# xiao-er-shang-jiu/Genie-TTS

Hardware: AMD Instinct MI355X
Metric: real-time factor + utterances/sec, 20-char JP, V2 speaker, 1/2/4/8 MI355X (higher is better)
Workload: dtype f32 activations (fp16-valued weights; split-fp16 MFMA GEMMs); 1 GPU; configs[1]: V2 speaker, single utterance, greedy, 1 utt per replica; a stream of such utterances, each one's vocoder on 64 CUs beside the next one's T2S; ref_phones=48, text_phones=45, ssl_frames=264, loop_steps=81, samples=102400, parallelism=replicas x1, vocoder_cus=64, streams_per_gpu=1, vits_f32_reruns=0

## Files before the change

genie_tts_amd/csrc/engine.hip:

```cpp
#include <hip/hip_runtime.h>
#include <hip/hip_fp16.h>

#include <chrono>
#include <cmath>
#include <cstdio>
#include <cstdlib>
#include <cstring>
#include <mutex>
#include <thread>
#include <map>
#include <memory>
#include <string>
#include <vector>

#include "../../include/genie_engine.h"
#include "engine_internal.h"
#include "kernels.h"
#include "prefill_attn.h"

using namespace gsv;

static thread_local std::string g_err;

const char* gsv_last_error(void) { return g_err.c_str(); }
// ... 265 lines not shown
}

int gsv_engine::finalize_t2s() {
    int err = 0;
    std::vector<float> div = default_div_term();
    if (const Staged* s = find("pe.div_term"))
        if (s->data.size() == 256) div = s->data;
    pe_max = 4096;
    if (const char* e = std::getenv("GENIE_FFN_SLICES")) ffn_slices = std::atoi(e) == 32 ? 32 : 64;
    if (const char* e = std::getenv("GENIE_ACC")) use_acc = std::atoi(e) != 0;
    if (const char* e = std::getenv("GENIE_PERSIST")) use_persist = std::atoi(e) != 0;
    if (const char* e = std::getenv("GENIE_PERSIST1")) use_persist1 = std::atoi(e) != 0;
    if (const char* e = std::getenv("GENIE_PERSIST1M")) use_persist1m = std::atoi(e) != 0;
    if (const char* e = std::getenv("GENIE_PERSISTM")) use_persistm = std::atoi(e) != 0;
    if (const char* e = std::getenv("GENIE_PRESPLIT")) use_presplit = std::atoi(e) != 0;
    if (const char* e = std::getenv("GENIE_CONVH")) use_convh = std::atoi(e) != 0;
    if (const char* e = std::getenv("GENIE_CONVH_WS")) convh_ws = std::max(0, std::min(2, std::atoi(e)));
    if (const char* e = std::getenv("GENIE_VITS_FORK")) vits_fork = std::atoi(e) != 0;
    if (const char* e = std::getenv("GENIE_PF_DELAY")) persist1_pf_delay = std::max(0, std::atoi(e));
    if (const char* e = std::getenv("GENIE_KTRACE"))
        if (std::atoi(e) == 1 && !ktrace) {
            hipMalloc(&ktrace, (size_t)3 * 256 * 8 * 8);
            hipMemset(ktrace, 0, (size_t)3 * 256 * 8 * 8);
        }
    std::vector<float> pe((size_t)pe_max * 512);
    for (int p = 0; p < pe_max; ++p)
        for (int i = 0; i < 256; ++i) {
            const float ang = (float)p * div[i];
            pe[(size_t)p * 512 + 2 * i] = std::sin(ang);
            pe[(size_t)p * 512 + 2 * i + 1] = std::cos(ang);
// ... 184 lines not shown
    e_h = A((size_t)cp * 768 * 4);
    e_hh = A((size_t)cp * 4);
    e_dist = A((size_t)cp * 1024 * 4);
    e_bproj = A((size_t)cl * 512 * 4);
    e_bert = A((size_t)cl * 1024 * 4);
    if (!e_im2col || !e_h || !e_hh || !e_dist || !e_bproj || !e_bert) return set_error(GSV_E_HIP, "encoder workspace");
    enc_cap_p = cp;
    enc_cap_l = cl;
    return 0;
}

int gsv_engine::encode(const gsv_utt* u, float* x, int64_t* prompts, hipStream_t st, bool do_prompts) {
    const int L = u->n_ref + u->n_text, P = u->n_ssl / 2;
    if (L <= 0 || P <= 0) return set_error(GSV_E_ARG, "empty utterance");
    if (int e = ensure_enc_ws(P, L)) return e;
    if (do_prompts) {
    ssl_im2col(u->ssl, u->n_ssl, e_im2col, st);
    GemmArgs g{};
    g.M = P; g.N = 768; g.K = 1536;
    g.A = e_im2col; g.lda = 1536;
    g.W = ssl_w; g.ldw = 1536; g.w_f16 = 0;
    g.bias = ssl_b; g.C = e_h; g.ldc = 768; g.mode = EPI_STORE;
    gemm_nt(g, st);
    sumsq_rows(e_h, 768, P, 768, e_hh, st);
    GemmArgs d{};
    d.M = P; d.N = 1024; d.K = 768;
    d.A = e_h; d.lda = 768; d.W = codebook; d.ldw = 768; d.w_f16 = 0;
    d.C = e_dist; d.ldc = 1024; d.mode = EPI_VQDIST; d.rowsq = e_hh; d.colsq = cb_sumsq;
    gemm_nt(d, st);
    argmin_dist_rows(e_dist, P, 1024, prompts, st);
    }
    const float* bproj = nullptr;
    if (u->ref_bert || u->text_bert) {
        if (u->ref_bert)
            hipMemcpyAsync(e_bert, u->ref_bert, (size_t)u->n_ref * 1024 * 4, hipMemcpyDeviceToDevice, st);
        else
            hipMemsetAsync(e_bert, 0, (size_t)u->n_ref * 1024 * 4, st);
        if (u->text_bert)
            hipMemcpyAsync(e_bert + (size_t)u->n_ref * 1024, u->text_bert, (size_t)u->n_text * 1024 * 4,
                           hipMemcpyDeviceToDevice, st);
        else
            hipMemsetAsync(e_bert + (size_t)u->n_ref * 1024, 0, (size_t)u->n_text * 1024 * 4, st);
        GemmArgs b{};
        b.M = L; b.N = 512; b.K = 1024;
        b.A = e_bert; b.lda = 1024; b.W = bert_w; b.ldw = 1024; b.w_f16 = 0;
        b.C = e_bproj; b.ldc = 512; b.mode = EPI_STORE;
        gemm_nt(b, st);
        bproj = e_bproj;
    }
    text_embed(u->ref_seq, u->n_ref, u->text_seq, u->n_text, text_emb, bproj, bert_b, alpha_text,
               pe_tab, x, st);
    const hipError_t le = hipGetLastError();
    return le == hipSuccess ? 0 : hip_error("encode launch", le);
}

int gsv_engine::prefill_slot(int b, const float* x, int L, const int64_t* pr, int P,
                             const gsv_sampler* sp, float* logits_out, hipStream_t st, int noise_b) {
    const int N0 = L + P;
    if (N0 + 1 > tmax) return set_error(GSV_E_CAPACITY, "prefill exceeds reserved tokens");
    if (x != pH) hipMemcpyAsync(pH, x, (size_t)L * 512 * 4, hipMemcpyDeviceToDevice, st);
    seq_state_init(b, pr, P, L, y, tmax, ny, kvlen, steps, done, seen, st);
    audio_embed_prompts(pr, P, emb_audio, alpha_audio, pe_tab, pH + (size_t)L * 512, st);
    hipLaunchKernelGGL(k_fill_row_len, dim3((N0 + 255) / 256), dim3(256), 0, st, prow_len, L, N0);
    const long sstride = (long)16 * tmax * 32;
    for (int l = 0; l < 24; ++l) {
        const T2SLayerW& W = layers[l];
        GemmArgs g{};
        g.M = N0; g.N = 1536; g.K = 512; g.A = pH; g.lda = 512;
        g.W = W.w_in; g.ldw = 512; g.w_f16 = 1; g.bias = W.b_in;
        g.C = pQ; g.ldc = 512; g.mode = EPI_QKV;
        g.kv.k = kcache[l] + b * sstride; g.kv.v = vcache[l] + b * sstride;
        g.kv.tmax = tmax; g.kv.pos0 = 0; g.kv.seq_stride = sstride;
        gemm_nt(g, st);
        AttnArgs at{};
        at.q = pQ; at.ldq = 512; at.k = kcache[l] + b * sstride; at.v = vcache[l] + b * sstride;
        at.seq_stride = sstride; at.tmax = tmax; at.row_len = prow_len; at.out = pO; at.ldo = 512;
        at.rows = N0; at.scale = qk_scale;
        attn_rows(at, st);
        const bool slabs = gemm_slabs_supported(512, 512, 512) && gemm_slabs_supported(2048, 2048, 2048);
        const long slab_stride = (long)tmax * 512;
        GemmArgs go{};
        go.M = N0; go.N = 512; go.K = 512; go.A = pO; go.lda = 512;
        go.W = W.w_out; go.ldw = 512; go.w_f16 = 1; go.bias = W.b_out;
        if (slabs) {
            go.C = pSlab; go.ldc = 512; go.mode = EPI_SLAB; go.ksplit = 4; go.slab_stride = slab_stride;
            gemm_nt(go, st);
            layernorm_rows_slabs(pSlab, 4, slab_stride, W.b_out, pH, pH1, N0, W.n1w, W.n1b, st);
        } else {
            go.C = pS; go.ldc = 512; go.mode = EPI_RESID; go.res = pH; go.ldr = 512;
            gemm_nt(go, st);
            layernorm_rows(pS, pH1, N0, W.n1w, W.n1b, st);
        }
        GemmArgs g1{};
        g1.M = N0; g1.N = 2048; g1.K = 512; g1.A = pH1; g1.lda = 512;
        g1.W = W.w1; g1.ldw = 512; g1.w_f16 = 1; g1.bias = W.b1;
        g1.C = pF; g1.ldc = 2048; g1.mode = EPI_RELU;
        gemm_nt(g1, st);
        GemmArgs g2{};
        g2.M = N0; g2.N = 512; g2.K = 2048; g2.A = pF; g2.lda = 2048;
        g2.W = W.w2; g2.ldw = 2048; g2.w_f16 = 1; g2.bias = W.b2;
        if (slabs) {
            g2.C = pSlab; g2.ldc = 512; g2.mode = EPI_SLAB; g2.ksplit = 8; g2.slab_stride = slab_stride;
            gemm_nt(g2, st);
            layernorm_rows_slabs(pSlab, 8, slab_stride, W.b2, pH1, pH, N0, W.n2w, W.n2b, st);
        } else {
            g2.C = pS; g2.ldc = 512; g2.mode = EPI_RESID; g2.res = pH1; g2.ldr = 512;
            gemm_nt(g2, st);
            layernorm_rows(pS, pH, N0, W.n2w, W.n2b, st);
        }
    }
    GemvArgs lg{};
    lg.B = 1; lg.N = 1025; lg.K = 512; lg.src = pH + (size_t)(N0 - 1) * 512; lg.lds = 512;
    lg.W = w_pred; lg.C = logits + (size_t)b * 1025; lg.ldc = 1025; lg.mode = EPI_STORE;
    gemv_f16(lg, st);
    SampleArgs sa = sampler_args(sp, 1);
// ... 1264 lines not shown
        if (value < 2) return set_error(GSV_E_ARG, "persistm_min_b: >= 2");
        eng->persistm_min_b = value;
    } else if (n == "persist_spin_ticks") {
        eng->persist_spin_ticks = value > 0 ? (unsigned long long)value : gsv_engine::PERSIST_SPIN_TICKS;
    } else if (n == "persist1_f16_limit") {
        eng->persist1_f16_limit = value;
    } else if (n == "pf_delay") {
        eng->persist1_pf_delay = std::max(0, value);
    } else if (n.size() == 5 && n.compare(0, 4, "knob") == 0 && n[4] >= '0' && n[4] <= '3') {
        eng->persist1_knob[n[4] - '0'] = value;
    } else if (n == "vits_lanes") {
        if (value < 1 || value > 16) return set_error(GSV_E_ARG, "vits_lanes: 1..16");
        eng->vits_lanes = value;
    } else if (n == "gemm_presplit") {
        eng->use_presplit = value != 0;
    } else if (n == "convh_ws") {
        eng->convh_ws = std::max(0, std::min(2, value));
    } else if (n == "vits_fork") {
        eng->vits_fork = value != 0;
    } else if (n == "vocoder_first") {
        eng->vocoder_first = value != 0;
    } else if (n == "lanes_all_cus") {
        if (int r = eng->vits_batch_finish(nullptr)) return r;
        eng->sync_own_streams();
        eng->lanes_all_cus = value != 0;
        if (int r = eng->remake_lane_streams()) return r;
    } else if (n == "lane_priority" || n == "t2s_priority") {
        int least = 0, greatest = 0;
        hipDeviceGetStreamPriorityRange(&least, &greatest);
        const int p = std::min(std::max(value, std::min(least, greatest)), std::max(least, greatest));
// ... 75 lines not shown
}

extern "C" int gsv_request_stop(gsv_engine* eng, int32_t on) {
    ENG_CHECK(eng);
    __atomic_store_n(eng->stop_word, on ? 1 : 0, __ATOMIC_RELEASE);
    return 0;
}

extern "C" int gsv_get_counter(gsv_engine* eng, const char* name, int64_t* value) {
    ENG_CHECK(eng);
    if (!name || !value) return set_error(GSV_E_ARG, "null arg");
    const std::string n(name);
    if (n == "persist_timeouts") *value = eng->persist_timeouts;
    else if (n == "persist1_f16_reruns") *value = eng->persist1_f16_reruns;
    else if (n == "vits_f32_reruns") *value = eng->vits_f32_reruns;
    else if (n == "vits_packed_fronts") *value = eng->vits_packed_fronts;
    else if (n == "sv_f32_reruns") *value = eng->sv_f32_reruns;
    else if (n == "w16_split_tensors") *value = eng->w16_split_tensors;
    else if (n == "persist_disabled") *value = eng->persist_disabled;
    else if (n == "persist_launches") *value = eng->persist_launches;
    else if (n == "decode_lanes") *value = eng->decode_lanes();
    else if (n == "lane_launches_0") *value = eng->lb.launches[0];
    else if (n == "lane_launches_1") *value = eng->lb.launches[1];
    else if (n == "persist_hold") *value = eng->persist_hold;
    else if (n == "stops") *value = eng->stops;
    else if (n == "graph_fallbacks") *value = eng->graph_fallbacks;
    else if (n == "retired_bytes") { std::lock_guard<std::mutex> g(eng->alloc_mu); *value = eng->retired_bytes; }
    else if (n == "reclaimed_bytes") *value = eng->reclaimed_bytes;
    else if (n == "reclaims") *value = eng->reclaims;
    else return set_error(GSV_E_ARG, "unknown counter " + n);
// ... 61 lines not shown
```

genie_tts_amd/csrc/engine_internal.h:

```cpp
#pragma once
#include <hip/hip_runtime.h>
#include <hip/hip_fp16.h>

#include <algorithm>
#include <map>
#include <mutex>
#include <shared_mutex>
#include <memory>
#include <thread>
#include <string>
#include <vector>

#include "../../include/genie_engine.h"
#include "kernels.h"
#include "lanes.h"
#include "vits.h"

namespace gsv {
int set_error(int code, const std::string& msg);
int check_sampler(const gsv_sampler* s);
inline float norm_top_p(float p) { return p == 0.f ? 1.f : p; }
int hip_error(const std::string& what, hipError_t e);
int f16_inexact_error(const std::string& weight, const float* v, int64_t index);
struct StreamScope;
// ... 192 lines not shown
    size_t sv_ws_floats(int frames);
    int sv_forward(const float* wav, int n, float* out, hipStream_t st, int* ovf, float lim);
    int roberta_forward(const int64_t* ids, int N, const int* rows, int n_out, float* out, hipStream_t st,
                        const int* row_pos = nullptr, const int* row_seg = nullptr);
    int reserve(int batch, int tokens);
    int ensure_enc_ws(int P, int L);
    int encode(const gsv_utt* u, float* x, int64_t* prompts, hipStream_t st, bool do_prompts = true);
    bool use_packed = true;
    bool use_attn_mf32 = true;
    int pk_rows = 0, pk_batch = 0;
    std::vector<void*> pk_allocs;
    float *pk_H = nullptr, *pk_Q = nullptr, *pk_O = nullptr, *pk_S = nullptr, *pk_H1 = nullptr, *pk_F = nullptr;
    float *pk_slab = nullptr, *pk_xlast = nullptr;
    __half *pk_Hh = nullptr, *pk_Hl = nullptr, *pk_H1h = nullptr, *pk_H1l = nullptr, *pk_Fh = nullptr, *pk_Fl = nullptr;
    bool use_presplit = true;
    int *pk_rowinfo = nullptr, *pk_last = nullptr;
    int64_t* pk_prompts = nullptr;
    int* pk_tiles = nullptr;
    int pk_tile_cap = 0;
    std::vector<int> pk_host;
    int ensure_packed(int rows, int B);
    int prefill_packed(int B, const gsv_utt* utts, const gsv_sampler* sp, hipStream_t st);
    int prefill_slot(int b, const float* x, int L, const int64_t* pr, int P, const gsv_sampler* sp,
                     float* logits_out, hipStream_t st, int noise_b = -1);
    gsv::SampleArgs sampler_args(const gsv_sampler* sp, int B);
    void decode_step(int B, const gsv_sampler* sp, float* logits_out, hipStream_t st);
    hipGraphExec_t step_graph(int B, const gsv_sampler* sp, int chunk, hipStream_t st);
    int decode_loop(int B, const gsv_sampler* sp, hipStream_t st, bool allow_persist = true);
    long persist_timeouts = 0;
    int persist_timeout_run = 0;
// ... 218 lines not shown
```

genie_tts_amd/csrc/kernels.h:

```cpp
#pragma once
#include <hip/hip_runtime.h>
#include <hip/hip_fp16.h>
#include <stdint.h>

namespace gsv {

enum EpiMode {
    EPI_STORE = 0,
    EPI_RELU = 1,
    EPI_RESID = 2,
    EPI_QKV = 3,
    EPI_VQDIST = 4,
    EPI_MISH = 5,
    EPI_SLAB = 6,
    EPI_GELU = 7,
    EPI_RELU_SPLIT = 8,
};

struct KVScatter {
    float* k;
    float* v;
    int tmax;
    int pos0;
    const int* row_pos;
// ... 12 lines not shown
struct GemmArgs {
    int M, N, K;
    const float* A; long lda;
    const void* W; long ldw; int w_f16;
    const void* Wl;
    const float* bias;
    float* C; long ldc;
    int mode;
    const float* res; long ldr;
    const float* rowsq; const float* colsq;
    KVScatter kv;
    int ksplit; long slab_stride;
    int a_nslab; long a_slab_stride; const float* a_bias; int a_relu;
    const __half* Ah; const __half* Al;
    __half* Ch; __half* Cl;
};
void gemm_nt(const GemmArgs& a, hipStream_t s);
GemmArgs gemm_f16(int M, int N, int K, const float* A, long lda, const void* W, const float* bias, float* C,
                  long ldc, int mode, const float* res = nullptr, long ldr = 0);
GemmArgs gemm_w16(int M, int N, int K, const float* A, long lda, const W16& W, const float* bias, float* C,
                  long ldc, int mode, const float* res = nullptr, long ldr = 0);
bool gemm_slabs_supported(int K, long lda, long ldw);
bool gemm_w16_supported(int K, long lda, long ldw);
bool gemm_presplit_path(int M, int N, int K, long lda);

void layernorm_rows(const float* in, float* out, int rows, const float* g, const float* b,
                    hipStream_t s);
void layernorm_rows_slabs(const float* slabs, int nsplit, long slab_stride, const float* bias,
                          const float* res, float* out, int rows, const float* g, const float* b,
                          hipStream_t s, __half* out_hi = nullptr, __half* out_lo = nullptr);
// ... 162 lines not shown
```

genie_tts_amd/csrc/t2s.hip:

```cpp
#include "common.h"
#include "kernels.h"
#include "prefill_attn.h"
#include "sampler.h"
#include <cstdio>
#include <cstdlib>

namespace gsv {

__device__ __forceinline__ void gemm_epilogue(const GemmArgs& a, int row0, int col, int lane, const f32x16& acc) {
    if (col >= a.N) return;
    const float bv = a.bias ? a.bias[col] : 0.f;
#pragma unroll
    for (int r = 0; r < 16; ++r) {
        const int row = row0 + (r & 3) + 8 * (r >> 2) + 4 * (lane >> 5);
        if (row >= a.M) continue;
        const float v = a.bias ? bv + acc[r] : acc[r];
        switch (a.mode) {
            case EPI_STORE: a.C[(long)row * a.ldc + col] = v; break;
            case EPI_RELU: a.C[(long)row * a.ldc + col] = fmaxf(v, 0.f); break;
            case EPI_RELU_SPLIT: {
                float x = fmaxf(v, 0.f);
                asm volatile("" : "+v"(x));
                const _Float16 h = (_Float16)x;
                reinterpret_cast<_Float16*>(a.Ch)[(long)row * a.ldc + col] = h;
// ... 343 lines not shown
        if (a.mode == EPI_SLAB) {
            if (col >= a.N) continue;
            float* C = a.C + (long)kz * a.slab_stride;
#pragma unroll
            for (int i = 0; i < 16; ++i) {
                const int row = m0 + wm * 32 + (i & 3) + 8 * (i >> 2) + 4 * hh;
                if (row < a.M) C[(long)row * a.ldc + col] = acc[t][i];
            }
            continue;
        }
        gemm_epilogue(a, m0 + wm * 32, col, lane, acc[t]);
    }
}

enum class X3Form { SplitW, LargeM, SmallM };
static void launch_x3(const GemmArgs& a, int z, hipStream_t s, X3Form form) {
    auto go = [&](auto kern) {
        hipLaunchKernelGGL(kern, dim3((a.N + 63) / 64, (a.M + 63) / 64, z), dim3(256), 0, s, a);
    };
    switch (form) {
        case X3Form::SplitW: go(k_gemm_x3<64, 64, 2, true, 1, true>); break;
        case X3Form::LargeM:
            if (a.Ah) go(k_gemm_x3<64, 64, 2, false, 1, true, true>);
            else go(k_gemm_x3<64, 64, 2, false, 1, true>);
            break;
        case X3Form::SmallM: go(k_gemm_x3<64, 64, 4>); break;
    }
}

static bool gemm_big(const GemmArgs& a) { return (long)((a.M + 63) / 64) * ((a.N + 63) / 64) >= 1024; }

bool gemm_w16_supported(int K, long lda, long ldw) { return K % GX_KS == 0 && lda % 4 == 0 && ldw % 8 == 0; }

bool gemm_presplit_path(int M, int N, int K, long lda) {
    if (K % GX_KS != 0 || lda % 8 != 0) return false;
    GemmArgs t{};
    t.M = M; t.N = N;
    return gemm_big(t);
}

bool gemm_slabs_supported(int K, long lda, long ldw) { return K % GX_KS == 0 && lda % 4 == 0 && ldw % 8 == 0; }
// ... 1010 lines not shown
```

genie_tts_amd/csrc/vits.h:

```cpp
#pragma once
#include <hip/hip_runtime.h>
#include <hip/hip_fp16.h>
#include <stdint.h>

#include <vector>

namespace gsv {

constexpr int MHA_MAXK_HOST = 2048;

enum ConvMode {
    CV_STORE = 0,
    CV_RELU = 1,
    CV_RESID = 2,
    CV_VEC = 3,
    CV_SUB = 4,
    CV_TANH = 5,
    CV_ACC_FIRST = 6,
    CV_ACC_ADD = 7,
    CV_ACC_MEAN = 8,
    CV_RESID_VEC = 9,
    CV_SPLIT_RESID = 10,
};

// ... 5 lines not shown
    int in_act; float in_slope;
    int mode;
    const float* res; long r_cs, r_ts;
    const float* vec;
    float* acc; float div;
    int split; float* out2; const float* res2;
    int phases; long w_phase_stride;
    float* part; long part_cap;
    const __half* wh; const float* wscale; int* ovf;
    long wh_phase_stride; const float* in_scale;
    const int* seg; long vec_sstride;
    int tile_force;
    int ws;
};
void conv1d(const ConvArgs& a, hipStream_t s);
void seg_fill(int* seg, long n, const int* off, const int* len, int nseg, int f, hipStream_t s);
bool conv1d_h(const ConvArgs& a, hipStream_t s);

struct MrfPairArgs {
    const float* r; int T, C, K, dil;
    const __half* w1; const float* s1; const float* b1;
    const __half* w2; const float* s2;
    int* ovf;
    ConvArgs e;
};
bool mrf_pair(const MrfPairArgs& a, hipStream_t s);

void mean3(const float* a, const float* b, const float* c, float* out, long n, float div, hipStream_t s);
void ln_channels(const float* x, const float* y, float* out, int C, int T, const float* g,
                 const float* b, hipStream_t s, const int* seg = nullptr);

struct MhaArgs {
    const float* q; long q_ts, q_cs;
    const float* k; long k_ts, k_cs;
    const float* v; long v_ts, v_cs;
    float* out; long o_ts, o_cs;
    int nq, nk, heads, dk;
    int postdiv; float scale;
    const float* ek; const float* ev; int window;
    const int* row_seg;
};
void mha(const MhaArgs& a, hipStream_t s);

void codebook_upsample2(const int64_t* sem, int G, const float* cb, float* out, hipStream_t s);
void embed_channels(const int64_t* ids, int n, const float* emb, int C, float* out, hipStream_t s);
void wn_gate(const float* xin, float* acts, int H, int T, hipStream_t s);
void glu_resid(const float* h, const float* x, float* out, int C, int T, long x_cs, long x_ts,
               hipStream_t s);
void noise_zp(const float* m, const float* logs, const float* eps, float scale, float* z, int n,
              hipStream_t s);
void noise_zp_philox(const float* m, const float* logs, uint64_t seed, float scale, float* z, int n,
                     hipStream_t s);
void flip_channels(const float* in, float* out, int C, int T, hipStream_t s);
void interp_linear(const float* x, int C, int T, int T_out, float* out, hipStream_t s);
void codebook_upsample2_seg(const int64_t* const* sems, const int* seg, const int* off, int T, const float* cb,
                            float* out, hipStream_t s);
void embed_channels_seg(const int64_t* const* ids, const int* seg, const int* off, int n, const float* emb, int C,
                        float* out, hipStream_t s);
void noise_zp_philox_seg(const float* m, const float* logs, const uint64_t* seeds, const int* seg, const int* off,
                         const int* len, float scale, float* z, int C, int T, hipStream_t s);
void gather_vecs(const float* const* ptrs, int n, int dim, float* out, hipStream_t s);
// ... 81 lines not shown
```

genie_tts_amd/csrc/vits.hip:

```cpp
#include "common.h"
#include "vits.h"
#include "vits_epi.h"
#include <algorithm>
#include <cstdlib>

namespace gsv {

template <int KT> struct ConvCfg {
    static constexpr int CI = KT == 1 ? 32 : KT == 2 ? 32 : KT <= 4 ? 16 : KT <= 7 ? 8 : 4;
    static constexpr int KC = CI * KT;
};

#define CONV_BN 64
#define CONV_BM 64
#define CONV_XW_MAX 128

template <int KT, bool V4>
__global__ __launch_bounds__(256) void k_conv1d(ConvArgs a) {
    constexpr int CI = ConvCfg<KT>::CI, KC = ConvCfg<KT>::KC;
    constexpr int NX = (CI * CONV_XW_MAX + 255) / 256;
    constexpr int NW = (CONV_BM * KC / 4 + 255) / 256;
    __shared__ float Xs[2][CI * CONV_XW_MAX];
    __shared__ float Ws[2][CONV_BM][KC + 1];
    const int tid = threadIdx.x, lane = tid & 63, w = tid >> 6;
// ... 135 lines not shown
    else hipLaunchKernelGGL((k_conv1d<KT, false>), grid, dim3(256), 0, s, a);
}

static int conv_ci(int K) {
    switch (K) {
        case 1: return ConvCfg<1>::CI;
        case 2: return ConvCfg<2>::CI;
        case 3: return ConvCfg<3>::CI;
        case 4: return ConvCfg<4>::CI;
        case 5: return ConvCfg<5>::CI;
        case 7: return ConvCfg<7>::CI;
        default: return ConvCfg<11>::CI;
    }
}

void conv1d(const ConvArgs& a, hipStream_t s) {
    if (a.wh && conv1d_h(a, s)) return;
    dim3 grid((a.n_t + CONV_BN - 1) / CONV_BN, (a.Cout + CONV_BM - 1) / CONV_BM,
              a.phases > 0 ? a.phases : 1);
    int nsplit = 1;
    const int blocks = (int)(grid.x * grid.y);
    if (a.part && a.phases <= 1 && blocks < 128) {
        const int nch = (a.Cin + conv_ci(a.K) - 1) / conv_ci(a.K);
        nsplit = std::min(nch, (256 + blocks - 1) / blocks);
        while (nsplit > 1 && (long)nsplit * a.Cout * a.n_t > a.part_cap) --nsplit;
    }
    if (nsplit > 1) grid.z = nsplit;
    switch (a.K) {
        case 1: launch_conv<1>(a, grid, s); break;
        case 2: launch_conv<2>(a, grid, s); break;
        case 3: launch_conv<3>(a, grid, s); break;
        case 4: launch_conv<4>(a, grid, s); break;
        case 5: launch_conv<5>(a, grid, s); break;
        case 7: launch_conv<7>(a, grid, s); break;
        case 11: launch_conv<11>(a, grid, s); break;
        default: return;
    }
    if (nsplit > 1) {
        const long n = (long)a.Cout * a.n_t;
        hipLaunchKernelGGL(k_conv_reduce, dim3((unsigned)((n + 255) / 256)), dim3(256), 0, s, a, nsplit);
    }
}

__global__ __launch_bounds__(256) void k_mean3(const float4* __restrict__ a, const float4* __restrict__ b,
                                                const float4* __restrict__ c, float4* __restrict__ o, long n4,
                                                float div) {
    const long i = (long)blockIdx.x * 256 + threadIdx.x;
    if (i >= n4) return;
    const float4 x = a[i], y = b[i], z = c[i];
    o[i] = make_float4(((x.x + y.x) + z.x) / div, ((x.y + y.y) + z.y) / div, ((x.z + y.z) + z.z) / div,
                       ((x.w + y.w) + z.w) / div);
}
__global__ __launch_bounds__(256) void k_mean3_tail(const float* a, const float* b, const float* c, float* o, long lo,
                                                     long n, float div) {
    const long i = lo + (long)blockIdx.x * 256 + threadIdx.x;
    if (i < n) o[i] = ((a[i] + b[i]) + c[i]) / div;
// ... 61 lines not shown
            const float d = v[i] - mean;
            q += d * d;
        }
    }
    red[cg][tl] = q;
    __syncthreads();
    const float den = sqrtf((red[0][tl] + red[1][tl] + red[2][tl] + red[3][tl]) / (float)C + 1e-5f);
    if (!ok) return;
#pragma unroll
    for (int i = 0; i < LNC_MAX; ++i) {
        const int c = cg + 4 * i;
        if (c < C) out[(long)c * T + t] = (v[i] - mean) / den * g[c] + b[c];
    }
}

__global__ __launch_bounds__(64) void k_ln_channels_w(const float* x, const float* y, float* out,
                                                     int C, int T, const float* g, const float* b,
                                                     const int* seg) {
    const int lane = threadIdx.x, tl = lane & 3, cg = lane >> 2;
    const int t = blockIdx.x * 4 + tl;
    const bool ok = t < T;
    const bool gap = ok && seg && seg[t] < 0;
    const int nc = C >> 4;
    float v[16];
    float s = 0.f;
#pragma unroll
    for (int i = 0; i < 16; ++i) {
        float xv = 0.f;
        if (i < nc && ok) {
            const long o = (long)(cg + 16 * i) * T + t;
            xv = x[o];
            if (y) xv = xv + y[o];
        }
        v[i] = xv;
        s += xv;
    }
#pragma unroll
    for (int o = 4; o < 64; o <<= 1) s += __shfl_xor(s, o, 64);
    const float mean = s / (float)C;
    float q = 0.f;
#pragma unroll
    for (int i = 0; i < 16; ++i)
        if (i < nc) {
            const float d = v[i] - mean;
            q += d * d;
        }
#pragma unroll
    for (int o = 4; o < 64; o <<= 1) q += __shfl_xor(q, o, 64);
    const float den = sqrtf(q / (float)C + 1e-5f);
    if (!ok) return;
#pragma unroll
    for (int i = 0; i < 16; ++i)
        if (i < nc) {
            const int c = cg + 16 * i;
            out[(long)c * T + t] = gap ? 0.f : (v[i] - mean) / den * g[c] + b[c];
        }
}

void ln_channels(const float* x, const float* y, float* out, int C, int T, const float* g,
                 const float* b, hipStream_t s, const int* seg) {
    if (C % 16 == 0 && C <= 256)
        hipLaunchKernelGGL(k_ln_channels_w, dim3((T + 3) / 4), dim3(64), 0, s, x, y, out, C, T, g, b, seg);
    else if (!seg)
        hipLaunchKernelGGL(k_ln_channels, dim3((T + 63) / 64), dim3(256), 0, s, x, y, out, C, T, g, b);
    else
        std::abort();
}

#define MHA_MAXK 2048
#define MHA_MAXD 128
#define MHA_MAXW 8
__global__ __launch_bounds__(256) void k_mha(MhaArgs a) {
    __shared__ float qs[MHA_MAXD];
    __shared__ float p[MHA_MAXK];
    __shared__ float red[16];
    __shared__ float part[2][MHA_MAXD];
    __shared__ float qe[2 * MHA_MAXW + 1];
    const int hd = blockIdx.x, i = blockIdx.y, tid = threadIdx.x;
    const int dk = a.dk, c0 = hd * dk;
    int nk = a.nk;
    const float* kb = a.k;
// ... 107 lines not shown
}
void embed_channels(const int64_t* ids, int n, const float* emb, int C, float* out, hipStream_t s) {
    hipLaunchKernelGGL(k_embed_ch, dim3((n + 127) / 128, C), dim3(128), 0, s, ids, n, emb, C, out);
}

__global__ void k_wn_gate(const float* xin, float* acts, int H, int T) {
    const long i = (long)blockIdx.x * blockDim.x + threadIdx.x;
    if (i >= (long)H * T) return;
    const float a = xin[i], b = xin[i + (long)H * T];
    acts[i] = tanhf(a) * (1.0f / (1.0f + expf(-b)));
}
void wn_gate(const float* xin, float* acts, int H, int T, hipStream_t s) {
    const long n = (long)H * T;
    hipLaunchKernelGGL(k_wn_gate, dim3((n + 255) / 256), dim3(256), 0, s, xin, acts, H, T);
}

__global__ void k_glu(const float* h, const float* x, float* out, int C, int T, long x_cs, long x_ts) {
    const long i = (long)blockIdx.x * blockDim.x + threadIdx.x;
    if (i >= (long)C * T) return;
    const int c = (int)(i / T), t = (int)(i - (long)c * T);
    const float a = h[i], b = h[i + (long)C * T];
    const long xi = (long)c * x_cs + (long)t * x_ts;
    out[xi] = x[xi] + a * (1.0f / (1.0f + expf(-b)));
}
void glu_resid(const float* h, const float* x, float* out, int C, int T, long x_cs, long x_ts,
               hipStream_t s) {
    const long n = (long)C * T;
    hipLaunchKernelGGL(k_glu, dim3((n + 255) / 256), dim3(256), 0, s, h, x, out, C, T, x_cs, x_ts);
}

// ... 178 lines not shown
```

genie_tts_amd/csrc/vits_engine.hip:

```cpp
#include <hip/hip_runtime.h>

#include <cmath>
#include <cstring>
#include <cstdlib>
#include <string>
#include <vector>

#include "engine_internal.h"

#include <thread>

using namespace gsv;

namespace {

std::vector<float> fold_wn(const Staged* v, const Staged* g) {
    const long o = v->dims[0];
    const long per = (long)v->data.size() / o;
    std::vector<float> w(v->data.size());
    for (long i = 0; i < o; ++i) {
        double s = 0;
        for (long j = 0; j < per; ++j) s += (double)v->data[i * per + j] * v->data[i * per + j];
        const float nrm = (float)std::sqrt(s);
        const float gg = g->data[i];
// ... 307 lines not shown
    a.x = x; a.x_cs = T; a.x_ts = 1; a.Cin = c.cin; a.Tin = T;
    a.w = c.w; a.Cout = c.cout; a.K = c.k; a.dil = 1; a.pad = (c.k - 1) / 2;
    a.bias = c.b;
    a.out = out; a.o_cs = T; a.o_ts = 1; a.n_t = T; a.o_tstride = 1; a.o_toff = 0; a.o_len = T;
    a.mode = mode; a.r_cs = T; a.r_ts = 1;
    a.phases = 1;
    a.tile_force = tls_convh_tile;
    a.ws = tls_convh_ws;
    if (tls_ovf && c.wh) { a.wh = c.wh; a.wscale = c.wscale; a.ovf = tls_ovf; }
    return a;
}

static void attn_encoder(gsv_engine* e, const std::vector<AttnLayer>& Ls, float* x, int T, float* qkv,
                         float* att, float* tmp, float* ffn, hipStream_t s, const int* seg = nullptr,
                         const int* rows = nullptr) {
    for (const AttnLayer& L : Ls) {
        conv1d(cargs(L.qkv, x, T, qkv, CV_STORE, seg), s);
        MhaArgs m{};
        m.q = qkv; m.q_ts = 1; m.q_cs = T;
        m.k = qkv + (size_t)192 * T; m.k_ts = 1; m.k_cs = T;
        m.v = qkv + (size_t)384 * T; m.v_ts = 1; m.v_cs = T;
        m.out = att; m.o_ts = 1; m.o_cs = T;
        m.nq = T; m.nk = T; m.heads = 2; m.dk = 96; m.postdiv = 0; m.scale = std::sqrt(96.0f);
        m.ek = L.ek; m.ev = L.ev; m.window = 4;
        m.row_seg = rows;
        mha(m, s);
        conv1d(cargs(L.o, att, T, tmp, CV_STORE, seg), s);
        ln_channels(x, tmp, x, 192, T, L.g1, L.b1, s, seg);
        conv1d(cargs(L.ffn1, x, T, ffn, CV_RELU, seg), s);
        conv1d(cargs(L.ffn2, ffn, T, tmp, CV_STORE, seg), s);
        ln_channels(x, tmp, x, 192, T, L.g2, L.b2, s, seg);
    }
}

static void run_ref_enc(VitsWorkspace& W, const RefEnc& R, const float* audio, int n, float* ge,
                        hipStream_t s) {
    const int padded = n + 2 * 704;
    const int F = (padded - 2048) / 640 + 1;
    reflect_pad(audio, n, 704, W.pad, s);
    GemmArgs g{};
    g.M = F; g.N = 1408; g.K = 2048; g.A = W.pad; g.lda = 640;
    g.W = R.dft; g.ldw = 2048; g.w_f16 = 0; g.C = W.reim; g.ldc = 1408; g.mode = EPI_STORE;
    gemm_nt(g, s);
    stft_mag(W.reim, F, 704, W.spec, s);
    GemmArgs l0{};
    l0.M = F; l0.N = 128; l0.K = 704; l0.A = W.spec; l0.lda = 704;
// ... 611 lines not shown
        a.x_cs = 1; a.x_ts = c.cin;
        a.o_cs = 1; a.o_ts = c.cout;
        conv1d(a, s);
    };
    float* gcond = fs ? fs->gcond : W.gcond;
    for (int fi = 3; fi >= 0; --fi) {
        const auto& fl = V.flows[fi];
        flip_channels(W.z, W.z2, 192, T, s);
        vec_conv(fl.cond, ge, gcond);
        conv1d(cargs(fl.pre, W.z2, T, W.fh, CV_STORE, sT), s);
        hipMemsetAsync(W.fskip, 0, (size_t)192 * T * 4, s);
        for (int l = 0; l < 4; ++l) {
            ConvArgs ci = cargs(fl.in_l[l], W.fh, T, W.fx, CV_VEC, sT);
            ci.vec = gcond + l * 384;
            ci.vec_sstride = fl.cond.cout;
            conv1d(ci, s);
            wn_gate(W.fx, W.fa, 192, T, s);
            if (l < 3) {
                ConvArgs rs = cargs(fl.rs[l], W.fa, T, W.fh, CV_SPLIT_RESID, sT);
                rs.res = W.fh; rs.split = 192; rs.out2 = W.fskip; rs.res2 = W.fskip;
                conv1d(rs, s);
            } else {
                ConvArgs rs = cargs(fl.rs[l], W.fa, T, W.fskip, CV_RESID, sT);
                rs.res = W.fskip;
                conv1d(rs, s);
            }
        }
        ConvArgs po = cargs(fl.post, W.fskip, T, W.z2 + (size_t)96 * T, CV_SUB, sT);
        po.res = W.z2 + (size_t)96 * T;
        conv1d(po, s);
        float* t = W.z; W.z = W.z2; W.z2 = t;
    }
// ... 603 lines not shown
```

Measured before the change: 119.0 utt/s.

## Fuse split-K conv reductions into LayerNorm and WN gate; CU-aware small-M GEMM staging

Split-K conv1d calls in the VITS attention encoder and flow WN layers can now defer their partial-slab reduction. New kernels sum the slabs, add the bias and apply LayerNorm or the tanh-sigmoid gate in one pass, which removes a separate reduce kernel launch and a round trip through the intermediate buffer. Separately, the small-M T2S prefill GEMMs now receive the stream's CU count and use a 2-stage pipeline instead of 4 when the block count exceeds the available CUs, with an env/knob override. The trade-offs are extra code paths and a different reduction order, which can change numerics slightly.

```diff
diff --git a/genie_tts_amd/csrc/engine.hip b/genie_tts_amd/csrc/engine.hip
--- a/genie_tts_amd/csrc/engine.hip
+++ b/genie_tts_amd/csrc/engine.hip
@@ -303,6 +303,11 @@
     if (const char* e = std::getenv("GENIE_PERSIST1M")) use_persist1m = std::atoi(e) != 0;
     if (const char* e = std::getenv("GENIE_PERSISTM")) use_persistm = std::atoi(e) != 0;
     if (const char* e = std::getenv("GENIE_PRESPLIT")) use_presplit = std::atoi(e) != 0;
+    if (const char* e = std::getenv("GENIE_GEMM_SMALL_NS")) {
+        const int v = std::atoi(e);
+        gemm_small_ns = v >= 2 && v <= 4 ? v : 0;
+    }
+    if (const char* e = std::getenv("GENIE_VITS_SLAB_FUSE")) vits_slab_fuse = std::atoi(e) != 0;
     if (const char* e = std::getenv("GENIE_CONVH")) use_convh = std::atoi(e) != 0;
     if (const char* e = std::getenv("GENIE_CONVH_WS")) convh_ws = std::max(0, std::min(2, std::atoi(e)));
     if (const char* e = std::getenv("GENIE_VITS_FORK")) vits_fork = std::atoi(e) != 0;
@@ -517,19 +522,20 @@
     const int L = u->n_ref + u->n_text, P = u->n_ssl / 2;
     if (L <= 0 || P <= 0) return set_error(GSV_E_ARG, "empty utterance");
     if (int e = ensure_enc_ws(P, L)) return e;
+    const int cus = stream_cus(st);
     if (do_prompts) {
     ssl_im2col(u->ssl, u->n_ssl, e_im2col, st);
     GemmArgs g{};
     g.M = P; g.N = 768; g.K = 1536;
     g.A = e_im2col; g.lda = 1536;
     g.W = ssl_w; g.ldw = 1536; g.w_f16 = 0;
-    g.bias = ssl_b; g.C = e_h; g.ldc = 768; g.mode = EPI_STORE;
+    g.bias = ssl_b; g.C = e_h; g.ldc = 768; g.mode = EPI_STORE; g.cus = cus;
     gemm_nt(g, st);
     sumsq_rows(e_h, 768, P, 768, e_hh, st);
     GemmArgs d{};
     d.M = P; d.N = 1024; d.K = 768;
     d.A = e_h; d.lda = 768; d.W = codebook; d.ldw = 768; d.w_f16 = 0;
-    d.C = e_dist; d.ldc = 1024; d.mode = EPI_VQDIST; d.rowsq = e_hh; d.colsq = cb_sumsq;
+    d.C = e_dist; d.ldc = 1024; d.mode = EPI_VQDIST; d.rowsq = e_hh; d.colsq = cb_sumsq; d.cus = cus;
     gemm_nt(d, st);
     argmin_dist_rows(e_dist, P, 1024, prompts, st);
     }
@@ -547,7 +553,7 @@
         GemmArgs b{};
         b.M = L; b.N = 512; b.K = 1024;
         b.A = e_bert; b.lda = 1024; b.W = bert_w; b.ldw = 1024; b.w_f16 = 0;
-        b.C = e_bproj; b.ldc = 512; b.mode = EPI_STORE;
+        b.C = e_bproj; b.ldc = 512; b.mode = EPI_STORE; b.cus = cus;
         gemm_nt(b, st);
         bproj = e_bproj;
     }
@@ -566,12 +572,14 @@
     audio_embed_prompts(pr, P, emb_audio, alpha_audio, pe_tab, pH + (size_t)L * 512, st);
     hipLaunchKernelGGL(k_fill_row_len, dim3((N0 + 255) / 256), dim3(256), 0, st, prow_len, L, N0);
     const long sstride = (long)16 * tmax * 32;
+    const int cus = stream_cus(st);
     for (int l = 0; l < 24; ++l) {
         const T2SLayerW& W = layers[l];
         GemmArgs g{};
         g.M = N0; g.N = 1536; g.K = 512; g.A = pH; g.lda = 512;
         g.W = W.w_in; g.ldw = 512; g.w_f16 = 1; g.bias = W.b_in;
         g.C = pQ; g.ldc = 512; g.mode = EPI_QKV;
+        g.cus = cus; g.small_ns = gemm_small_ns;
         g.kv.k = kcache[l] + b * sstride; g.kv.v = vcache[l] + b * sstride;
         g.kv.tmax = tmax; g.kv.pos0 = 0; g.kv.seq_stride = sstride;
         gemm_nt(g, st);
@@ -585,6 +593,7 @@
         GemmArgs go{};
         go.M = N0; go.N = 512; go.K = 512; go.A = pO; go.lda = 512;
         go.W = W.w_out; go.ldw = 512; go.w_f16 = 1; go.bias = W.b_out;
+        go.cus = cus; go.small_ns = gemm_small_ns;
         if (slabs) {
             go.C = pSlab; go.ldc = 512; go.mode = EPI_SLAB; go.ksplit = 4; go.slab_stride = slab_stride;
             gemm_nt(go, st);
@@ -598,10 +607,12 @@
         g1.M = N0; g1.N = 2048; g1.K = 512; g1.A = pH1; g1.lda = 512;
         g1.W = W.w1; g1.ldw = 512; g1.w_f16 = 1; g1.bias = W.b1;
         g1.C = pF; g1.ldc = 2048; g1.mode = EPI_RELU;
+        g1.cus = cus; g1.small_ns = gemm_small_ns;
         gemm_nt(g1, st);
         GemmArgs g2{};
         g2.M = N0; g2.N = 512; g2.K = 2048; g2.A = pF; g2.lda = 2048;
         g2.W = W.w2; g2.ldw = 2048; g2.w_f16 = 1; g2.bias = W.b2;
+        g2.cus = cus; g2.small_ns = gemm_small_ns;
         if (slabs) {
             g2.C = pSlab; g2.ldc = 512; g2.mode = EPI_SLAB; g2.ksplit = 8; g2.slab_stride = slab_stride;
             gemm_nt(g2, st);
@@ -1896,6 +1907,11 @@
         eng->vits_lanes = value;
     } else if (n == "gemm_presplit") {
         eng->use_presplit = value != 0;
+    } else if (n == "vits_slab_fuse") {
+        eng->vits_slab_fuse = value != 0;
+    } else if (n == "gemm_small_ns") {
+        if (value != 0 && (value < 2 || value > 4)) return set_error(GSV_E_ARG, "gemm_small_ns: 0, 2, 3 or 4");
+        eng->gemm_small_ns = value;
     } else if (n == "convh_ws") {
         eng->convh_ws = std::max(0, std::min(2, value));
     } else if (n == "vits_fork") {
@@ -2001,6 +2017,7 @@
     if (n == "persist_timeouts") *value = eng->persist_timeouts;
     else if (n == "persist1_f16_reruns") *value = eng->persist1_f16_reruns;
     else if (n == "vits_f32_reruns") *value = eng->vits_f32_reruns;
+    else if (n == "vits_slab_consumers") *value = eng->vits_slab_consumers.load();
     else if (n == "vits_packed_fronts") *value = eng->vits_packed_fronts;
     else if (n == "sv_f32_reruns") *value = eng->sv_f32_reruns;
     else if (n == "w16_split_tensors") *value = eng->w16_split_tensors;
diff --git a/genie_tts_amd/csrc/engine_internal.h b/genie_tts_amd/csrc/engine_internal.h
--- a/genie_tts_amd/csrc/engine_internal.h
+++ b/genie_tts_amd/csrc/engine_internal.h
@@ -1,4 +1,5 @@
 #pragma once
+#include <atomic>
 #include <hip/hip_runtime.h>
 #include <hip/hip_fp16.h>
 
@@ -230,6 +231,9 @@
     float *pk_slab = nullptr, *pk_xlast = nullptr;
     __half *pk_Hh = nullptr, *pk_Hl = nullptr, *pk_H1h = nullptr, *pk_H1l = nullptr, *pk_Fh = nullptr, *pk_Fl = nullptr;
     bool use_presplit = true;
+    std::atomic<long> vits_slab_consumers{0};
+    bool vits_slab_fuse = true;
+    int gemm_small_ns = 0;
     int *pk_rowinfo = nullptr, *pk_last = nullptr;
     int64_t* pk_prompts = nullptr;
     int* pk_tiles = nullptr;
diff --git a/genie_tts_amd/csrc/kernels.h b/genie_tts_amd/csrc/kernels.h
--- a/genie_tts_amd/csrc/kernels.h
+++ b/genie_tts_amd/csrc/kernels.h
@@ -50,6 +50,7 @@
     int a_nslab; long a_slab_stride; const float* a_bias; int a_relu;
     const __half* Ah; const __half* Al;
     __half* Ch; __half* Cl;
+    int cus, small_ns;
 };
 void gemm_nt(const GemmArgs& a, hipStream_t s);
 GemmArgs gemm_f16(int M, int N, int K, const float* A, long lda, const void* W, const float* bias, float* C,
diff --git a/genie_tts_amd/csrc/t2s.hip b/genie_tts_amd/csrc/t2s.hip
--- a/genie_tts_amd/csrc/t2s.hip
+++ b/genie_tts_amd/csrc/t2s.hip
@@ -381,6 +381,12 @@
 }
 
 enum class X3Form { SplitW, LargeM, SmallM };
+
+static int small_m_stages(const GemmArgs& a, long blocks) {
+    if (a.small_ns) return a.small_ns;
+    return a.cus > 0 && blocks > a.cus ? 2 : 4;
+}
+
 static void launch_x3(const GemmArgs& a, int z, hipStream_t s, X3Form form) {
     auto go = [&](auto kern) {
         hipLaunchKernelGGL(kern, dim3((a.N + 63) / 64, (a.M + 63) / 64, z), dim3(256), 0, s, a);
@@ -391,7 +397,16 @@
             if (a.Ah) go(k_gemm_x3<64, 64, 2, false, 1, true, true>);
             else go(k_gemm_x3<64, 64, 2, false, 1, true>);
             break;
-        case X3Form::SmallM: go(k_gemm_x3<64, 64, 4>); break;
+        case X3Form::SmallM:
+            switch (small_m_stages(a, (long)((a.N + 63) / 64) * ((a.M + 63) / 64) * z)) {
+                case 2: go(k_gemm_x3<64, 64, 2>); break;
+                case 3: go(k_gemm_x3<64, 64, 3>); break;
+                case 4: go(k_gemm_x3<64, 64, 4>); break;
+                default:
+                    std::fprintf(stderr, "gemm_nt: small-M ring depth %d\n", a.small_ns);
+                    std::abort();
+            }
+            break;
     }
 }
 
diff --git a/genie_tts_amd/csrc/vits.h b/genie_tts_amd/csrc/vits.h
--- a/genie_tts_amd/csrc/vits.h
+++ b/genie_tts_amd/csrc/vits.h
@@ -43,6 +43,7 @@
     int ws;
 };
 void conv1d(const ConvArgs& a, hipStream_t s);
+int conv1d_deferred(const ConvArgs& a, hipStream_t s);
 void seg_fill(int* seg, long n, const int* off, const int* len, int nseg, int f, hipStream_t s);
 bool conv1d_h(const ConvArgs& a, hipStream_t s);
 
@@ -58,6 +59,8 @@
 void mean3(const float* a, const float* b, const float* c, float* out, long n, float div, hipStream_t s);
 void ln_channels(const float* x, const float* y, float* out, int C, int T, const float* g,
                  const float* b, hipStream_t s, const int* seg = nullptr);
+void ln_channels_slabs(const float* x, const float* slabs, int nsplit, const float* bias, float* out, int C, int T,
+                       const float* g, const float* b, hipStream_t s, const int* seg = nullptr);
 
 struct MhaArgs {
     const float* q; long q_ts, q_cs;
@@ -74,6 +77,8 @@
 void codebook_upsample2(const int64_t* sem, int G, const float* cb, float* out, hipStream_t s);
 void embed_channels(const int64_t* ids, int n, const float* emb, int C, float* out, hipStream_t s);
 void wn_gate(const float* xin, float* acts, int H, int T, hipStream_t s);
+void wn_gate_slabs(const float* slabs, int nsplit, const float* bias, const float* vec, long vec_sstride,
+                   const int* seg, float* acts, int H, int T, hipStream_t s);
 void glu_resid(const float* h, const float* x, float* out, int C, int T, long x_cs, long x_ts,
                hipStream_t s);
 void noise_zp(const float* m, const float* logs, const float* eps, float scale, float* z, int n,
diff --git a/genie_tts_amd/csrc/vits.hip b/genie_tts_amd/csrc/vits.hip
--- a/genie_tts_amd/csrc/vits.hip
+++ b/genie_tts_amd/csrc/vits.hip
@@ -173,8 +173,8 @@
     }
 }
 
-void conv1d(const ConvArgs& a, hipStream_t s) {
-    if (a.wh && conv1d_h(a, s)) return;
+static int conv1d_run(const ConvArgs& a, hipStream_t s, bool defer) {
+    if (a.wh && conv1d_h(a, s)) return 1;
     dim3 grid((a.n_t + CONV_BN - 1) / CONV_BN, (a.Cout + CONV_BM - 1) / CONV_BM,
               a.phases > 0 ? a.phases : 1);
     int nsplit = 1;
@@ -193,12 +193,20 @@
         case 5: launch_conv<5>(a, grid, s); break;
         case 7: launch_conv<7>(a, grid, s); break;
         case 11: launch_conv<11>(a, grid, s); break;
-        default: return;
-    }
-    if (nsplit > 1) {
+        default: return 1;
+    }
+    if (nsplit > 1 && !defer) {
         const long n = (long)a.Cout * a.n_t;
         hipLaunchKernelGGL(k_conv_reduce, dim3((unsigned)((n + 255) / 256)), dim3(256), 0, s, a, nsplit);
     }
+    return nsplit;
+}
+
+void conv1d(const ConvArgs& a, hipStream_t s) { conv1d_run(a, s, false); }
+
+int conv1d_deferred(const ConvArgs& a, hipStream_t s) {
+    const int nsplit = conv1d_run(a, s, true);
+    return nsplit > 1 ? nsplit : 0;
 }
 
 __global__ __launch_bounds__(256) void k_mean3(const float4* __restrict__ a, const float4* __restrict__ b,
@@ -290,6 +298,34 @@
     }
 }
 
+__device__ __forceinline__ void ln_w_finish(const float (&v)[16], float* out, int C, int T, const float* g,
+                                            const float* b, int t, int cg, bool ok, bool gap, int i0, int di) {
+    const int nc = C >> 4;
+    float s = 0.f;
+#pragma unroll
+    for (int i = 0; i < 16; ++i) s += v[i];
+#pragma unroll
+    for (int o = 4; o < 64; o <<= 1) s += __shfl_xor(s, o, 64);
+    const float mean = s / (float)C;
+    float q = 0.f;
+#pragma unroll
+    for (int i = 0; i < 16; ++i)
+        if (i < nc) {
+            const float d = v[i] - mean;
+            q += d * d;
+        }
+#pragma unroll
+    for (int o = 4; o < 64; o <<= 1) q += __shfl_xor(q, o, 64);
+    const float den = sqrtf(q / (float)C + 1e-5f);
+    if (!ok) return;
+#pragma unroll
+    for (int i = 0; i < 16; ++i)
+        if (i < nc && i % di == i0) {
+            const int c = cg + 16 * i;
+            out[(long)c * T + t] = gap ? 0.f : (v[i] - mean) / den * g[c] + b[c];
+        }
+}
+
 __global__ __launch_bounds__(64) void k_ln_channels_w(const float* x, const float* y, float* out,
                                                      int C, int T, const float* g, const float* b,
                                                      const int* seg) {
@@ -299,7 +335,6 @@
     const bool gap = ok && seg && seg[t] < 0;
     const int nc = C >> 4;
     float v[16];
-    float s = 0.f;
 #pragma unroll
     for (int i = 0; i < 16; ++i) {
         float xv = 0.f;
@@ -309,28 +344,58 @@
             if (y) xv = xv + y[o];
         }
         v[i] = xv;
-        s += xv;
-    }
-#pragma unroll
-    for (int o = 4; o < 64; o <<= 1) s += __shfl_xor(s, o, 64);
-    const float mean = s / (float)C;
-    float q = 0.f;
-#pragma unroll
-    for (int i = 0; i < 16; ++i)
-        if (i < nc) {
-            const float d = v[i] - mean;
-            q += d * d;
-        }
-#pragma unroll
-    for (int o = 4; o < 64; o <<= 1) q += __shfl_xor(q, o, 64);
-    const float den = sqrtf(q / (float)C + 1e-5f);
-    if (!ok) return;
-#pragma unroll
-    for (int i = 0; i < 16; ++i)
-        if (i < nc) {
-            const int c = cg + 16 * i;
-            out[(long)c * T + t] = gap ? 0.f : (v[i] - mean) / den * g[c] + b[c];
-        }
+    }
+    ln_w_finish(v, out, C, T, g, b, t, cg, ok, gap, 0, 1);
+}
+
+__global__ __launch_bounds__(256) void k_ln_channels_ws(const float* x, const float* slabs, int nsplit,
+                                                        const float* bias, float* out, int C, int T,
+                                                        const float* g, const float* b, const int* seg) {
+    __shared__ float vs[16][64];
+    const int lane = threadIdx.x & 63, w = threadIdx.x >> 6, tl = lane & 3, cg = lane >> 2;
+    const int t = blockIdx.x * 4 + tl;
+    const bool ok = t < T;
+    const bool gap = ok && seg && seg[t] < 0;
+    const int nc = C >> 4;
+    const long n = (long)C * T;
+    float xa[4], ya[4];
+#pragma unroll
+    for (int k = 0; k < 4; ++k) {
+        const int i = w + 4 * k;
+        xa[k] = ya[k] = 0.f;
+        if (i < nc && ok) xa[k] = x[(long)(cg + 16 * i) * T + t];
+    }
+    for (int s0 = 0; s0 < nsplit; s0 += 8) {
+        float p[4][8];
+#pragma unroll
+        for (int k = 0; k < 4; ++k) {
+            const int i = w + 4 * k;
+            const long o = (long)(cg + 16 * i) * T + t;
+#pragma unroll
+            for (int j = 0; j < 8; ++j)
+                p[k][j] = (i < nc && ok && s0 + j < nsplit) ? slabs[(long)(s0 + j) * n + o] : 0.f;
+        }
+#pragma unroll
+        for (int k = 0; k < 4; ++k)
+#pragma unroll
+            for (int j = 0; j < 8; ++j)
+                if (s0 + j < nsplit) ya[k] = (s0 + j == 0) ? p[k][j] : ya[k] + p[k][j];
+    }
+#pragma unroll
+    for (int k = 0; k < 4; ++k) {
+        const int i = w + 4 * k;
+        float xv = 0.f;
+        if (i < nc && ok) {
+            const float y = bias ? bias[cg + 16 * i] + ya[k] : ya[k];
+            xv = xa[k] + y;
+        }
+        vs[i][lane] = xv;
+    }
+    __syncthreads();
+    float v[16];
+#pragma unroll
+    for (int i = 0; i < 16; ++i) v[i] = vs[i][lane];
+    ln_w_finish(v, out, C, T, g, b, t, cg, ok, gap, w, 4);
 }
 
 void ln_channels(const float* x, const float* y, float* out, int C, int T, const float* g,
@@ -341,6 +406,13 @@
         hipLaunchKernelGGL(k_ln_channels, dim3((T + 63) / 64), dim3(256), 0, s, x, y, out, C, T, g, b);
     else
         std::abort();
+}
+
+void ln_channels_slabs(const float* x, const float* slabs, int nsplit, const float* bias, float* out, int C, int T,
+                       const float* g, const float* b, hipStream_t s, const int* seg) {
+    if (C % 16 != 0 || C > 256 || nsplit < 2) std::abort();
+    hipLaunchKernelGGL(k_ln_channels_ws, dim3((T + 3) / 4), dim3(256), 0, s, x, slabs, nsplit, bias, out, C, T, g,
+                       b, seg);
 }
 
 #define MHA_MAXK 2048
@@ -478,6 +550,46 @@
     const long n = (long)H * T;
     hipLaunchKernelGGL(k_wn_gate, dim3((n + 255) / 256), dim3(256), 0, s, xin, acts, H, T);
 }
+__global__ __launch_bounds__(256) void k_wn_gate_slabs(const float* slabs, int nsplit, const float* bias,
+                                                       const float* vec, long vec_sstride, const int* seg,
+                                                       float* acts, int H, int T) {
+    const long i = (long)blockIdx.x * 256 + threadIdx.x;
+    const long hn = (long)H * T;
+    if (i >= hn) return;
+    const int co = (int)(i / T), t = (int)(i - (long)co * T);
+    if (seg) {
+        const int sg = seg[t];
+        if (sg < 0) {
+            acts[i] = 0.f;
+            return;
+        }
+        vec += (long)sg * vec_sstride;
+    }
+    float sa = 0.f, sb = 0.f;
+    for (int s0 = 0; s0 < nsplit; s0 += 8) {
+        float pa[8], pb[8];
+#pragma unroll
+        for (int j = 0; j < 8; ++j) {
+            pa[j] = s0 + j < nsplit ? slabs[(long)(s0 + j) * 2 * hn + i] : 0.f;
+            pb[j] = s0 + j < nsplit ? slabs[(long)(s0 + j) * 2 * hn + hn + i] : 0.f;
+        }
+#pragma unroll
+        for (int j = 0; j < 8; ++j)
+            if (s0 + j < nsplit) {
+                sa = (s0 + j == 0) ? pa[j] : sa + pa[j];
+                sb = (s0 + j == 0) ? pb[j] : sb + pb[j];
+            }
+    }
+    const float va = bias ? bias[co] + sa : sa, vb = bias ? bias[co + H] + sb : sb;
+    const float a = va + vec[co], b = vb + vec[co + H];
+    acts[i] = tanhf(a) * (1.0f / (1.0f + expf(-b)));
+}
+void wn_gate_slabs(const float* slabs, int nsplit, const float* bias, const float* vec, long vec_sstride,
+                   const int* seg, float* acts, int H, int T, hipStream_t s) {
+    const long n = (long)H * T;
+    hipLaunchKernelGGL(k_wn_gate_slabs, dim3((unsigned)((n + 255) / 256)), dim3(256), 0, s, slabs, nsplit, bias, vec,
+                       vec_sstride, seg, acts, H, T);
+}
 
 __global__ void k_glu(const float* h, const float* x, float* out, int C, int T, long x_cs, long x_ts) {
     const long i = (long)blockIdx.x * blockDim.x + threadIdx.x;
diff --git a/genie_tts_amd/csrc/vits_engine.hip b/genie_tts_amd/csrc/vits_engine.hip
--- a/genie_tts_amd/csrc/vits_engine.hip
+++ b/genie_tts_amd/csrc/vits_engine.hip
@@ -345,6 +345,15 @@
 static void attn_encoder(gsv_engine* e, const std::vector<AttnLayer>& Ls, float* x, int T, float* qkv,
                          float* att, float* tmp, float* ffn, hipStream_t s, const int* seg = nullptr,
                          const int* rows = nullptr) {
+    auto conv_ln = [&](const Conv& c, const float* in, const float* g, const float* b) {
+        const ConvArgs a = cargs(c, in, T, tmp, CV_STORE, seg);
+        int ns = 0;
+        if (e->vits_slab_fuse) ns = conv1d_deferred(a, s);
+        else conv1d(a, s);
+        if (ns) ++e->vits_slab_consumers;
+        if (ns) ln_channels_slabs(x, a.part, ns, a.bias, x, 192, T, g, b, s, seg);
+        else ln_channels(x, tmp, x, 192, T, g, b, s, seg);
+    };
     for (const AttnLayer& L : Ls) {
         conv1d(cargs(L.qkv, x, T, qkv, CV_STORE, seg), s);
         MhaArgs m{};
@@ -356,11 +365,9 @@
         m.ek = L.ek; m.ev = L.ev; m.window = 4;
         m.row_seg = rows;
         mha(m, s);
-        conv1d(cargs(L.o, att, T, tmp, CV_STORE, seg), s);
-        ln_channels(x, tmp, x, 192, T, L.g1, L.b1, s, seg);
+        conv_ln(L.o, att, L.g1, L.b1);
         conv1d(cargs(L.ffn1, x, T, ffn, CV_RELU, seg), s);
-        conv1d(cargs(L.ffn2, ffn, T, tmp, CV_STORE, seg), s);
-        ln_channels(x, tmp, x, 192, T, L.g2, L.b2, s, seg);
+        conv_ln(L.ffn2, ffn, L.g2, L.b2);
     }
 }
 
@@ -1002,8 +1009,12 @@
             ConvArgs ci = cargs(fl.in_l[l], W.fh, T, W.fx, CV_VEC, sT);
             ci.vec = gcond + l * 384;
             ci.vec_sstride = fl.cond.cout;
-            conv1d(ci, s);
-            wn_gate(W.fx, W.fa, 192, T, s);
+            int ns = 0;
+            if (vits_slab_fuse) ns = conv1d_deferred(ci, s);
+            else conv1d(ci, s);
+            if (ns) ++vits_slab_consumers;
+            if (ns) wn_gate_slabs(ci.part, ns, ci.bias, ci.vec, ci.vec_sstride, ci.seg, W.fa, 192, T, s);
+            else wn_gate(W.fx, W.fa, 192, T, s);
             if (l < 3) {
                 ConvArgs rs = cargs(fl.rs[l], W.fa, T, W.fh, CV_SPLIT_RESID, sT);
                 rs.res = W.fh; rs.split = 192; rs.out2 = W.fskip; rs.res2 = W.fskip;
```

Result: faster. 125.2 utt/s (median of 6 runs) (+5.2%).
